# aelmiger/LINE-MOD-Pipeline

Hardware: AMD Instinct MI355X
Metric: detections/sec (higher is better)
Workload: dtype u8

## Files before the change

### line-mod-pipeline_amd/csrc/lm_common.h

```cpp
#pragma once
#include <stdint.h>

typedef uint8_t u8;
typedef uint16_t u16;
typedef uint32_t u32;
typedef uint64_t u64;

#define LM_SCAN_CHUNK 1008
#define LM_SCAN4_CHUNK 1016
#define LM_SCAN_FPAD 8
#define LM_SCANL_LDS_BYTES 163840
#define LM_SCANL_IMAGE_MAX 153600
#define LM_SCANL_TABLE_BYTES 2048
#define LM_SCANL_POS_BITS 15
#define LM_SORT_CAP 4096
#define LM_SORT_CHUNK 1024
#define LM_INLINE_MATCHES 2048
#define LM_DROPPED 0xFFFFFFFFu

#define PD_STRIP 16
#define CB_ROWS 2
#define CBS_STRIP 16
#define MX_WAVE_BYTES 128
#define CVT_ROWS 4
#define CG_STRIP 16
#define CT_W 32
#define CT_H 8
#define DT_W 64
#define DT_H 8
#define DM_ROWS 4
#ifndef DM_ROWS_BATCH
#define DM_ROWS_BATCH 16
#endif
#define LMK_MAX_LOADS 8

struct LmPhaseGrid { u32 nb[4]; int g[4]; };

struct LmLevelGeom {
    int w, h;
    int T;
    int W, H;
    int spread_only;
    int nibble;
    u32 wh;
    u32 ori_stride;
    u32 plane_ori;
    u32 mod_stride;
    u32 zero_off;
    u32 arena_bytes;
};

struct LmCand {
    u32 ti;
    int x, y;
    float sim;
};

struct LmRefFeat {
    u32 off;
    int16_t x, y;
};

struct LmRefMeta {
    int width, height;
    int nfeat_total;
// ... 55 lines not shown
```

### line-mod-pipeline_amd/csrc/lm_dev_depth.h

```cpp
#pragma once
#include "lm_dev.h"
#include "lm_median25.h"
#include "lm_median_counts.h"

namespace {

#define N_W (DT_W + 4)
#define N_H (DT_H + 4)
#define D_W (DT_W + 14)
#define D_H (DT_H + 14)
#define D_PITCH 80
#define D_LOADS ((D_H * D_W + 255) / 256)

typedef unsigned short us2 __attribute__((ext_vector_type(2)));
#define LM_CE(a, b) { us2 t_ = __builtin_elementwise_min(a, b); b = __builtin_elementwise_max(a, b); a = t_; }

__global__ __launch_bounds__(256) void k_depth_quantize(const u16* __restrict__ depth0, int w, int h, int dist_thr,
                                                         int diff_thr, const u8* __restrict__ lut,
                                                         u8* __restrict__ quant0, size_t slot_stride) {
    __shared__ u16 dt[D_H][D_PITCH];
    __shared__ u8 nt[N_H][N_W + 4];
    const u16* depth = slot_ptr(depth0, slot_stride);
    u8* quant = slot_ptr(quant0, slot_stride);
    const int tid = threadIdx.x;
// ... 197 lines not shown
    nx = nx * inv; ny = ny * inv; nz = nz * inv;
    const f32x2 t1 = nx * 10.f + 10.f, t2 = ny * 10.f + 10.f, t3 = nz * 20.f + 20.f;
    const u32 flat0 = (u32)mad_i24((int)t3[0], 400, mad_i24((int)t2[0], 20, (int)t1[0]));
    const u32 flat1 = (u32)mad_i24((int)t3[1], 400, mad_i24((int)t2[1], 20, (int)t1[1]));
    const u32 c0 = (u32)__builtin_amdgcn_raw_buffer_load_b8(lut_rsrc, (int)(LMK_NORMAL_CODE_OFFSET + min(flat0, 8000u)), 0, 0);
    const u32 c1 = (u32)__builtin_amdgcn_raw_buffer_load_b8(lut_rsrc, (int)(LMK_NORMAL_CODE_OFFSET + min(flat1, 8000u)), 0, 0);
    e0 = ok0 ? c0 : 0u; e1 = ok1 ? c1 : 0u;
}

__global__ __launch_bounds__(256) void k_selftest_float_tail(unsigned long long* __restrict__ out) {
    const u32 lo = 0x3F800000u, hi_rcp = (127u + 42u) << 23, hi_sqrt = (127u + 84u) << 23;
    unsigned long long bad_rcp = 0, bad_sqrt = 0, bad_bare = 0, c_rcp7 = 0, c_sqrt9 = 0, c_sqrt4 = 0, c_inv = 0;
    for (u32 b = lo + blockIdx.x * 256u + threadIdx.x; b <= hi_sqrt; b += gridDim.x * 256u) {
        const float x = __builtin_bit_cast(float, b);
        if (b <= hi_rcp) bad_rcp += __builtin_bit_cast(u32, dn_rcp(x)) != __builtin_bit_cast(u32, __fdiv_rn(1.0f, x));
        const u32 want = __builtin_bit_cast(u32, __builtin_sqrtf(x));
        bad_sqrt += __builtin_bit_cast(u32, dn_sqrt(x)) != want;
        bad_bare += __builtin_bit_cast(u32, dn_sqrt_bare(x)) != want;
        if (b <= hi_rcp) c_rcp7 += __builtin_bit_cast(u32, dn_rcp7(x)) != __builtin_bit_cast(u32, __fdiv_rn(1.0f, x));
        c_sqrt9 += __builtin_bit_cast(u32, dn_sqrt9(x)) != want;
        c_sqrt4 += __builtin_bit_cast(u32, dn_sqrt4(x)) != want;
        c_inv += __builtin_bit_cast(u32, dn_inv_from_rsq(x, dn_sqrt(x))) != __builtin_bit_cast(u32, __fdiv_rn(1.0f, __builtin_sqrtf(x)));
    }
    if (blockIdx.x == 0 && threadIdx.x == 0) bad_sqrt += dn_sqrt(0.0f) > 0.0f ? 1u : 0u;
    if (bad_rcp) atomicAdd(&out[0], bad_rcp);
    if (bad_sqrt) atomicAdd(&out[1], bad_sqrt);
    if (bad_bare) atomicAdd(&out[2], bad_bare);
    if (c_rcp7) atomicAdd(&out[3], c_rcp7);
    if (c_sqrt9) atomicAdd(&out[4], c_sqrt9);
    if (c_sqrt4) atomicAdd(&out[5], c_sqrt4);
    if (c_inv) atomicAdd(&out[6], c_inv);
}

template <bool SMALL>
__device__ __forceinline__ void d_dnormal_t(const u32 vblock, const u16* __restrict__ depth0, int w, int h, int dist_thr, int diff_thr,
                                                  const u8* __restrict__ lut, u8* __restrict__ code0, size_t in_stride,
                                                  size_t tmp_stride, int gblocks, int nslots) {
    u32 slot, tile;
    xcd_slot_tile_b(vblock, (u32)gblocks, (u32)nslots, slot, tile);
    const u16* depth = slot_ptr_s(depth0, in_stride, slot);
    u8* code = slot_ptr_s(code0, tmp_stride, slot);
    const int ng = w >> 3;
    const int gid = (int)(tile * 256u) + (int)threadIdx.x;
    const int y = gid / ng, g = gid - y * ng;
    if (y >= h) return;
    u32 out[2] = {0, 0};
    if (y >= 5 && y < h - 6) {
        u32x4 R[3][3];
#pragma unroll
        for (int j = 0; j < 3; ++j) {
            const u8* row = reinterpret_cast<const u8*>(depth + (size_t)(y + 5 * (j - 1)) * w) + 16 * g - 16;
#pragma unroll
            for (int k = 0; k < 3; ++k) {
                const bool ok = !(k == 0 && g == 0) && !(k == 2 && g == ng - 1);
                R[j][k] = ok ? ld16(row + 16 * k) : u32x4{0, 0, 0, 0};
            }
        }
        if (diff_thr >= 0 && diff_thr <= 5461) {
            const __amdgpu_buffer_rsrc_t lut_rsrc = __builtin_amdgcn_make_buffer_rsrc(const_cast<u8*>(lut), 0, 2 * 8000 + 16, 0x00020000);
            u32 D[3][12];
#pragma unroll
            for (int j = 0; j < 3; ++j)
#pragma unroll
                for (int k = 0; k < 12; ++k) D[j][k] = R[j][k >> 2][k & 3];
            const u32 THR = (u32)diff_thr * 0x00010001u;
#pragma unroll
            for (int k = 0; k < 4; ++k) {
                const u32 C = D[1][4 + k];
                u32 F[3][3], G[3][3];
#pragma unroll
                for (int jj = -1; jj <= 1; ++jj)
#pragma unroll
                    for (int ii = -1; ii <= 1; ++ii) {
                        if (ii == 0 && jj == 0) continue;
                        const u32* Dr = D[jj + 1];
                        const u32 N = ii == 0 ? Dr[4 + k]
                                    : ii > 0 ? __builtin_amdgcn_alignbit(Dr[7 + k], Dr[6 + k], 16)
                                             : __builtin_amdgcn_alignbit(Dr[2 + k], Dr[1 + k], 16);
                        const u32 up = pk_sub_u16_sat(N, C), dn = pk_sub_u16_sat(C, N);
                        const u32 f = pk_min_u16(pk_sub_u16_sat(THR, up | dn), 0x00010001u);
                        F[jj + 1][ii + 1] = f;
                        G[jj + 1][ii + 1] = pk_mul_lo_u16(pk_sub_i16(up, dn), f);
                    }
                const u32 fdp = F[2][2] + F[0][0], fdm = F[2][0] + F[0][2];
                const u32 cd = fdp + fdm;
                const u32 cx = pk_sub_i16(fdp, fdm);
                const u32 ci = F[1][2] + F[1][0] + cd, cj = F[2][1] + F[0][1] + cd;
                const u32 ga = pk_sub_i16(G[2][2], G[0][0]), gb = pk_sub_i16(G[0][2], G[2][0]);
                const u32 sx = pk_add_i16(pk_add_i16(pk_sub_i16(G[1][2], G[1][0]), ga), gb);
                const u32 sy = pk_sub_i16(pk_add_i16(pk_sub_i16(G[2][1], G[0][1]), ga), gb);
                const u32 ncx = pk_sub_i16(0u, cx);
                const int d0 = (int)(C & 0xFFFFu), d1 = (int)(C >> 16);
                const int detq0 = mad_i16h<false>(ci, cj, mad_i16h<false>(ncx, cx, 0)), detq1 = mad_i16h<true>(ci, cj, mad_i16h<true>(ncx, cx, 0));
                const int ddxq0 = mad_i16h<false>(cj, sx, mad_i16h<false>(ncx, sy, 0)), ddxq1 = mad_i16h<true>(cj, sx, mad_i16h<true>(ncx, sy, 0));
                const int ddyq0 = mad_i16h<false>(ci, sy, mad_i16h<false>(ncx, sx, 0)), ddyq1 = mad_i16h<true>(ci, sy, mad_i16h<true>(ncx, sx, 0));
                u32 e0, e1;
                dn_label2<SMALL>(detq0, ddxq0, ddyq0, d0, d0 < dist_thr, detq1, ddxq1, ddyq1, d1, d1 < dist_thr, lut_rsrc, e0, e1);
                out[k >> 1] |= (e0 | (e1 << 8)) << (16 * (k & 1));
            }
        } else {
#pragma unroll
        for (int p = 0; p < 8; ++p) {
            const int d = (int)hw_u16(R[1], 8 + p);
            const bool valid = d < dist_thr;
            int ci = 0, cj = 0, cx = 0, sx = 0, sy = 0;
#pragma unroll
            for (int jj = -1; jj <= 1; ++jj)
#pragma unroll
                for (int ii = -1; ii <= 1; ++ii) {
                    if (ii == 0 && jj == 0) continue;
                    const int delta = (int)hw_u16(R[jj + 1], 8 + p + 5 * ii) - d;
                    const int ad = delta < 0 ? -delta : delta;
                    const int f = ad < diff_thr ? 1 : 0;
                    const int fd = ad < diff_thr ? delta : 0;
                    if (ii != 0) { ci += f; sx += ii * fd; }
                    if (jj != 0) { cj += f; sy += jj * fd; }
                    if (ii != 0 && jj != 0) cx += ii * jj * f;
                }
            const int A0 = 25 * ci, A3 = 25 * cj, A1 = 25 * cx, b0 = 5 * sx, b1 = 5 * sy;
            const int det = mul_i24(A0, A3) - mul_i24(A1, A1);
            const int ddx = mul_i24(A3, b0) - mul_i24(A1, b1);
            const int ddy = mul_i24(A0, b1) - mul_i24(A1, b0);
            const u32 e = dn_label<false>(det, ddx, ddy, d, valid, lut);
            out[p >> 2] |= e << (8 * (p & 3));
        }
        }
    }
    {
        const int xlo = 5 - 8 * g, xhi = (w - 6) - 8 * g;
        unsigned long long m = ~0ull;
        if (xlo > 0) m &= xlo >= 8 ? 0ull : (~0ull << (8 * xlo));
        if (xhi < 8) m &= xhi <= 0 ? 0ull : (~0ull >> (8 * (8 - xhi)));
        out[0] &= (u32)m; out[1] &= (u32)(m >> 32);
    }
    *reinterpret_cast<u32x2*>(code + (size_t)y * w + 8 * g) = u32x2{out[0], out[1]};
}
__device__ __forceinline__ void d_dnormal(const u32 vblock, const u16* __restrict__ depth0, int w, int h, int dist_thr, int diff_thr,
                                          const u8* __restrict__ lut, u8* __restrict__ code0, size_t in_stride,
                                          size_t tmp_stride, int gblocks, int nslots) {
    if (diff_thr >= 0 && diff_thr <= 249) d_dnormal_t<true>(vblock, depth0, w, h, dist_thr, diff_thr, lut, code0, in_stride, tmp_stride, gblocks, nslots);
    else d_dnormal_t<false>(vblock, depth0, w, h, dist_thr, diff_thr, lut, code0, in_stride, tmp_stride, gblocks, nslots);
}
__global__ __launch_bounds__(256) void k_dnormal(const u16* __restrict__ depth0, int w, int h, int dist_thr, int diff_thr,
                                                  const u8* __restrict__ lut, u8* __restrict__ code0, size_t in_stride,
                                                  size_t tmp_stride, int gblocks, int nslots) {
    d_dnormal(blockIdx.x, depth0, w, h, dist_thr, diff_thr, lut, code0, in_stride, tmp_stride, gblocks, nslots);
}

template <int ROWS>
__device__ __forceinline__ void d_dmedian(const u32 vblock, const u8* __restrict__ code0, int w, int h, u8* __restrict__ quant0,
                                                  size_t tmp_stride, size_t out_stride, int gblocks, int nslots) {
    u32 slot, tile;
    xcd_slot_tile_b(vblock, (u32)gblocks, (u32)nslots, slot, tile);
    const u8* code = slot_ptr_s(code0, tmp_stride, slot);
    u8* quant = slot_ptr_s(quant0, out_stride, slot);
    const int ng = w >> 3;
    const int gid = (int)(tile * 256u) + (int)threadIdx.x;
    const int band = gid / ng, g = gid - band * ng;
    const int y0 = band * ROWS;
    if (y0 >= h) return;
    u32 ring[5][8];
#pragma unroll
    for (int i = 0; i < ROWS + 4; ++i) {
        const int yy = clampi(y0 - 2 + i, 0, h - 1);
        const u32 ro = (u32)yy * (u32)w + 8u * (u32)g;
        const u8* row = code + ro;
        const u32x2 c = *reinterpret_cast<const u32x2*>(row);
        u32 e[12];
#pragma unroll
        for (int k = 0; k < 8; ++k) e[2 + k] = (c[k >> 2] >> (8 * (k & 3))) & 0xFFu;
        const u32 l = *reinterpret_cast<const u32*>(code + (g > 0 ? ro - 4u : ro)), r = *reinterpret_cast<const u32*>(code + (g + 1 < ng ? ro + 8u : ro + 4u));
        e[0] = g > 0 ? (l >> 16) & 0xFFu : e[2]; e[1] = g > 0 ? l >> 24 : e[2];
        e[10] = g + 1 < ng ? r & 0xFFu : e[9]; e[11] = g + 1 < ng ? (r >> 8) & 0xFFu : e[9];
        u32 cw[12];
#pragma unroll
        for (int k = 0; k < 12; ++k) cw[k] = lm_mc_word(e[k]);
        u32 t3[10];
#pragma unroll
        for (int k = 0; k < 10; ++k) t3[k] = cw[k] + cw[k + 1] + cw[k + 2];
// ... 26 lines not shown
```

### line-mod-pipeline_amd/csrc/lm_host.cpp

```cpp
#include "lm_host.h"
#if defined(__x86_64__)
#include <immintrin.h>
#endif

#include <algorithm>
#include <atomic>
#include <cassert>
#include <cmath>
#include <cstdio>
#include <cstdlib>
#include <cstring>

namespace lmh {

int Bank::find(const std::string& id) const {
    for (size_t i = 0; i < classes.size(); ++i)
        if (classes[i].id == id) return (int)i;
    return -1;
}

int Bank::add_pyramid(const std::string& id, TemplatePyramid&& tp) {
    int ci = find(id);
    if (ci < 0) { classes.push_back(ClassEntry{id, {}}); ci = (int)classes.size() - 1; }
    classes[ci].pyramids.push_back(std::move(tp));
// ... 952 lines not shown
    const bool dep = in.M == 2;
    const int g_blur0 = cblur_blocks(w, h), g_blur1 = cblur_blocks(w1, h1);
    const int g_ori0 = corient_blocks(w, h), g_ori1 = corient_blocks(w1, h1);
    const int g_vote0 = cvote_blocks(w, h), g_vote1 = cvote_blocks(w1, h1);
    const int g_pyr = pyrdown8_blocks(w, h), g_nrm = dnormal_blocks(w, h), g_med = dmedian_blocks(w, h, DM_ROWS);
    const int seg0 = T0 == 5 ? lm_fast_segs(w / 5, 128) : lm_spread2_blocks(w, h), seg1 = lm_fast_segs(w1 / 8, 40);
    const u32 b_lm0 = T0 == 5 ? (u32)(seg0 * (h / 5) * n) : (u32)(seg0 * n), b_lm1 = (u32)(seg1 * (h1 / 8) * n);
    add_fused(p, K::Phase1, {{(u32)(g_blur0 * n), dep ? (u32)(g_nrm * n) : 0u, (u32)(g_pyr * n), 0u}, {g_blur0, g_nrm, g_pyr, 0}});
    add_fused(p, K::Phase2, {{dep ? (u32)(g_med * n) : 0u, (u32)(g_blur1 * n), (u32)(g_ori0 * n), 0u}, {g_med, g_blur1, g_ori0, 0}});
    add_fused(p, K::Phase3, {{(u32)(g_vote0 * n), (u32)(g_ori1 * n), dep ? b_lm0 : 0u, dep ? b_lm1 : 0u}, {g_vote0, g_ori1, seg0, seg1}});
    add_fused(p, T0 == 5 ? K::Phase4_T5 : K::Phase4_T2, {{(u32)(g_vote1 * n), b_lm0, 0u, 0u}, {g_vote1, seg0, 0, 0}});
    plan_mode_lm_fast(p, K::LmFast8_40, 40, 1, 0, false, in);
}

bool batch_phases_shape(const PreInputs& in) {
    if (!phases_shape(in) || !batch(in)) return false;
    if (in.lv[0].T == 5) return (in.lv[0].w % 5) == 0 && spread5_shape(in, 0, 0) && (in.M < 2 || spread5_shape(in, 0, 1));
    return in.M < 2;
}
void plan_batch_phases(const PreInputs& in, PrePlan& p) {
    const PreLevel &v0 = in.lv[0], &v1 = in.lv[1];
    const int w = v0.w, h = v0.h, w1 = w / 2, h1 = h / 2, n = in.n, T0 = v0.T;
    const bool tall = h > 640;
    const int sb = cblur_sh_strip(h);
    const int sg = tall ? 32 : 16;
    const int g_nrm = dnormal_blocks(w, h), g_blur0 = cblur_sh_blocks(w, h, sb), g_pyr = pyrdown16_blocks(w, h);
    const int g_grad0 = cgrad_blocks(w, h, sg), g_med = dmedian_blocks(w, h, DM_ROWS_BATCH), g_blur1 = cblur_sh_blocks(w1, h1, 16);
    const int g_grad1 = cgrad_blocks(w1, h1, 16);
    const int g_sp = T0 == 5 ? lm_spread5_blocks(w, h) : lm_spread2_blocks(w, h);
    const int seg1 = lm_fast_segs(w1 / 8, 40);
    const u32 b_lm1 = (u32)(seg1 * (h1 / 8) * n);
    if (in.M == 2) {
        if (plan_blur_pyrdown(in, p)) {
            add_slots(p, K::Dnormal, 0, 1, g_nrm, in);
        } else {
            add_fused(p, K::Bsplit0, {{(u32)(g_nrm * n), (u32)(g_pyr * n), 0u, 0u}, {g_nrm, g_pyr, 0, 0}});
            add_slots(p, tall ? K::CblurSh32 : K::CblurSh16, 0, 0, g_blur0, in);
        }
        add_fused(p, tall ? K::Bsplit1_32 : K::Bsplit1_16, {{(u32)(g_grad0 * n), (u32)(g_blur1 * n), 0u, 0u}, {g_grad0, g_blur1, 0, 0}});
        add_slots(p, K::Dmedian16, 0, 1, g_med, in);
        const int s1 = cgrad_strip_upper(w1, h1, n);
        add_slots(p, cgrad_kernel(s1), 1, 0, cgrad_blocks(w1, h1, s1), in);
        add_fused(p, K::Bsplit2, {{(u32)(g_sp * n), (u32)(g_sp * n), b_lm1, 0u}, {g_sp, g_sp, seg1, 0}});
    } else {
        const bool bp = plan_blur_pyrdown(in, p);
        static const K table[2][2][3] = {{{K::Bphase1_T5_16, K::Bphase2_T5_16, K::Bphase3_T5_16}, {K::Bphase1_T5_32, K::Bphase2_T5_32, K::Bphase3_T5_32}},
                                         {{K::Bphase1_T2_16, K::Bphase2_T2_16, K::Bphase3_T2_16}, {K::Bphase1_T2_32, K::Bphase2_T2_32, K::Bphase3_T2_32}}};
        const auto kern = [&](int ph) { return table[T0 == 5 ? 0 : 1][tall ? 1 : 0][ph - 1]; };
        if (!bp) add_fused(p, kern(1), {{0u, (u32)(g_blur0 * n), (u32)(g_pyr * n), 0u}, {g_nrm, g_blur0, g_pyr, 0}});
        add_fused(p, kern(2), {{(u32)(g_grad0 * n), 0u, (u32)(g_blur1 * n), 0u}, {g_grad0, g_med, g_blur1, 0}});
        add_fused(p, kern(3), {{(u32)(g_grad1 * n), (u32)(g_sp * n), 0u, 0u}, {g_grad1, g_sp, g_sp, seg1}});
    }
    const bool wide = lm_fast8_wide(w1 / 8, h1, v1.mode, v1.a_lm[0], in.a_stride, in.ori_stride, in.planes);
    plan_mode_lm_fast(p, wide ? K::LmFast8_80 : K::LmFast8_40, wide ? 80 : 40, 1, 0, false, in);
}

}

void plan_pyrdown(const PreInputs& in, int l, PrePlan& p) {
    const int sw = in.lv[l - 1].w, sh = in.lv[l - 1].h, v = in.knobs.pyrdown_variant;
    if (v != 1 && (v == 2 || batch(in)) && pyrdown16_shape(in, l)) add_slots(p, K::Pyrdown16, l, 0, pyrdown16_blocks(sw, sh), in);
    else if (pyrdown_streams(in, l)) add_slots(p, K::Pyrdown8, l, 0, pyrdown8_blocks(sw, sh), in);
    else add_tiles(p, K::Pyrdown, l, 0, pre_ceil(sw / 2, 64), pre_ceil(sh / 2, 4), in);
}

void plan_nn_half(const PreInputs& in, int l, PrePlan& p) { add_tiles(p, K::NnHalf, l, 1, pre_ceil(in.lv[l].w, 64), pre_ceil(in.lv[l].h, 4), in); }

void plan_color_quantize(const PreInputs& in, int l, bool blurred, PrePlan& p) {
    const int w = in.lv[l].w, h = in.lv[l].h, v = in.knobs.cgrad_variant;
    if (!color_streams(in, l)) { add_tiles(p, K::ColorQuantize, l, 0, pre_ceil(w, CT_W), pre_ceil(h, CT_H), in); return; }
    if (!blurred) add_blur(in, l, pick_blur(in, l), p);
    if (!in.want_mag && (v >= 2 || (v == 0 && batch(in)))) {
        const int strip = cgrad_strip(w, h, in.n, v == 3);
        add_slots(p, cgrad_kernel(strip), l, 0, cgrad_blocks(w, h, strip), in);
        return;
    }
    add_slots(p, K::Corient, l, 0, corient_blocks(w, h), in);
    add_slots(p, K::Cvote, l, 0, cvote_blocks(w, h), in);
}

void plan_depth_quantize(const PreInputs& in, PrePlan& p) {
    const int w = in.lv[0].w, h = in.lv[0].h, v = in.knobs.dmedian_variant;
    if (!depth_streams(in)) { add_tiles(p, K::DepthQuantize, 0, 1, pre_ceil(w, DT_W), pre_ceil(h, DT_H), in); return; }
    const bool dm_batch = v == 2 || (v == 0 && batch(in));
    add_slots(p, K::Dnormal, 0, 1, dnormal_blocks(w, h), in);
    add_slots(p, dm_batch ? K::Dmedian16 : K::Dmedian4, 0, 1, dmedian_blocks(w, h, dm_batch ? DM_ROWS_BATCH : DM_ROWS), in);
}

void plan_linear_memories(const PreInputs& in, int l, int m, u32 planes, PrePlan& p) {
    const PreLevel& v = in.lv[l];
    const bool sh = m != 0 && l != 0;
    const int w = v.w, h = v.h, T = v.T, W = w / T, mode = v.mode;
    const int qpitch = sh ? in.lv[l - 1].w : w;
    const u32 a_q = sh ? in.lv[l - 1].a_quant[1] : v.a_quant[m], a_lm = v.a_lm[m];
    if ((w % 4) == 0 && (W % 4) == 0 && (qpitch % 4) == 0 && (a_q & 3) == 0 && (in.a_stride & 3) == 0) {
        switch (T) {
            case 2:
                if (mode == 1 && !sh && (w % 32) == 0 && (h % 2) == 0 && (qpitch % 16) == 0 && a_q == 0 && a_lm == 0 && in.a_stride == 0 && (((size_t)W * (h / 2)) % 16) == 0) {
                    add_slots(p, K::LmSpread2, l, m, lm_spread2_blocks(w, h), in);
                    return;
                }
                plan_mode_lm_fast(p, K::LmFast2_128, 128, l, m, sh, in); return;
            case 4: plan_mode_lm_fast(p, K::LmFast4_64, 64, l, m, sh, in); return;
            case 5:
                if (mode == 1 && !sh && batch(in) && spread5_shape(in, l, m)) { add_slots(p, K::LmSpread5, l, m, lm_spread5_blocks(w, h), in); return; }
                plan_mode_lm_fast(p, K::LmFast5_128, 128, l, m, sh, in); return;
            case 8: {
                const bool wide = lm_fast8_wide(W, h, mode, a_lm, in.a_stride, in.ori_stride, planes);
                plan_mode_lm_fast(p, wide ? K::LmFast8_80 : K::LmFast8_40, wide ? 80 : 40, l, m, sh, in); return;
            }
            default: break;
        }
    }
    int seg = (1024 / (T * T)) & ~3;
    if (seg < 4) seg = 4;
    while (seg > 4 && (2 * T - 1) * (seg * T + T - 1) > LMK_MAX_LOADS * 256) seg -= 4;
    if (seg > W) seg = (W + 3) & ~3;
    const int pitch = (seg * T + T + 3) & ~3;
// ... 76 lines not shown
```

### line-mod-pipeline_amd/csrc/lm_k_preprocess.hip

```cpp
#include "lm_dev_color.h"
#include "lm_dev_depth.h"
#include "lm_dev_memories.h"
#include "lm_host.h"

namespace {

template <int PH, int T0>
__global__ __launch_bounds__(256) void k_phase(LmPhaseArgs a, LmPhaseGrid pg) {
    const u32 b = blockIdx.x, e0 = pg.nb[0], e1 = e0 + pg.nb[1], e2 = e1 + pg.nb[2];
    const size_t fs = a.slot_stride;
    const int w1 = a.w >> 1, h1 = a.h >> 1;
    const size_t a3_0 = ((size_t)a.w * a.h * 3 + 255) / 256 * 256, a3_1 = ((size_t)w1 * h1 * 3 + 255) / 256 * 256;
    const float thr2 = a.weak_threshold * a.weak_threshold;
    if (PH == 1) {
        if (b < e0) d_cblur(b, a.bgr0, a.w, a.h, a.cs0, fs, fs, pg.g[0], a.nslots);
        else if (b < e1) d_dnormal(b - e0, a.depth, a.w, a.h, a.dist_thr, a.diff_thr, a.normal_lut, a.ds, fs, fs, pg.g[1], a.nslots);
        else d_pyrdown8(b - e1, a.bgr0, a.w, a.h, a.bgr1, w1, h1, fs, pg.g[2], a.nslots);
    } else if (PH == 2) {
        if (b < e0) d_dmedian<DM_ROWS>(b, a.ds, a.w, a.h, a.qd0, fs, fs, pg.g[0], a.nslots);
        else if (b < e1) d_cblur(b - e0, a.bgr1, w1, h1, a.cs1, fs, fs, pg.g[1], a.nslots);
        else d_corient(b - e1, a.cs0, a.w, a.h, thr2, a.cs0 + a3_0, nullptr, fs, fs, pg.g[2], a.nslots);
    } else if (PH == 3) {
        if (b < e0) d_cvote(b, a.cs0 + a3_0, a.w, a.h, a.qc0, fs, fs, pg.g[0], a.nslots);
        else if (b < e1) d_corient(b - e0, a.cs1, w1, h1, thr2, a.cs1 + a3_1, nullptr, fs, fs, pg.g[1], a.nslots);
        else if (b < e2) d_lm_fast<5, 128, 0, 1>(b - e1, a.qd0, a.w, a.w, a.h, a.resp_tab, a.lm_d0, 0u, fs, fs, pg.g[2], a.nslots);
        else d_lm_fast<8, 40, 1, 2>(b - e2, a.qd0, a.w, w1, h1, a.resp_tab, a.lm_d1, a.ori_stride1, fs, fs, pg.g[3], a.nslots, a.plane_ori1);
    } else {
        if (b < e0) d_cvote(b, a.cs1 + a3_1, w1, h1, a.qc1, fs, fs, pg.g[0], a.nslots);
        else if (T0 == 5) d_lm_fast<5, 128, 0, 1>(b - e0, a.qc0, a.w, a.w, a.h, a.resp_tab, a.lm_c0, 0u, fs, fs, pg.g[1], a.nslots);
        else d_lm_spread2(b - e0, a.qc0, a.w, a.w, a.h, a.lm_c0, fs, fs, pg.g[1], a.nslots);
    }
}

template <int PH, int T0, int SB, int SG>
__global__ __launch_bounds__(256, 2) void k_bphase(LmPhaseArgs a, LmPhaseGrid pg) {
    const u32 b = blockIdx.x, e0 = pg.nb[0], e1 = e0 + pg.nb[1], e2 = e1 + pg.nb[2];
    const size_t fs = a.slot_stride;
    const int w1 = a.w >> 1, h1 = a.h >> 1, n = a.nslots;
    const float thr2 = a.weak_threshold * a.weak_threshold;
    const int ithr = thr2 >= 2147483648.f ? INT_MAX : (int)floorf(thr2);
    if (PH == 1) {
        if (b < e0) d_dnormal(b, a.depth, a.w, a.h, a.dist_thr, a.diff_thr, a.normal_lut, a.ds, fs, fs, pg.g[0], n);
        else if (b < e1) d_cblur_sh<SB>(b - e0, a.bgr0, a.w, a.h, a.cs0, fs, fs, pg.g[1], n);
        else d_pyrdown16<PD_STRIP>(b - e1, a.bgr0, a.w, a.h, a.bgr1, w1, h1, fs, pg.g[2], n);
    } else if (PH == 2) {
        if (b < e0) d_cgrad<SG>(b, a.cs0, a.w, a.h, ithr, a.qc0, fs, fs, pg.g[0], n);
        else if (b < e1) d_dmedian<DM_ROWS_BATCH>(b - e0, a.ds, a.w, a.h, a.qd0, fs, fs, pg.g[1], n);
        else d_cblur_sh<16>(b - e1, a.bgr1, w1, h1, a.cs1, fs, fs, pg.g[2], n);
    } else {
        if (b < e0) d_cgrad<16>(b, a.cs1, w1, h1, ithr, a.qc1, fs, fs, pg.g[0], n);
        else if (b < e1) {
            if (T0 == 5) d_lm_spread5(b - e0, a.qc0, a.w, a.w, a.h, a.lm_c0, fs, fs, pg.g[1], n);
            else d_lm_spread2(b - e0, a.qc0, a.w, a.w, a.h, a.lm_c0, fs, fs, pg.g[1], n);
        }
        else if (b < e2) d_lm_spread5(b - e1, a.qd0, a.w, a.w, a.h, a.lm_d0, fs, fs, pg.g[2], n);
        else d_lm_fast<8, 40, 1, 2>(b - e2, a.qd0, a.w, w1, h1, a.resp_tab, a.lm_d1, a.ori_stride1, fs, fs, pg.g[3], n, a.plane_ori1);
    }
}

template <int PART, int SG>
__global__ __launch_bounds__(256, PART == 1 ? 2 : 1) void k_bsplit(LmPhaseArgs a, LmPhaseGrid pg) {
    const u32 b = blockIdx.x, e0 = pg.nb[0], e1 = e0 + pg.nb[1];
    const size_t fs = a.slot_stride;
    const int w1 = a.w >> 1, h1 = a.h >> 1, n = a.nslots;
    if (PART == 0) {
        if (b < e0) d_dnormal(b, a.depth, a.w, a.h, a.dist_thr, a.diff_thr, a.normal_lut, a.ds, fs, fs, pg.g[0], n);
        else d_pyrdown16<PD_STRIP>(b - e0, a.bgr0, a.w, a.h, a.bgr1, w1, h1, fs, pg.g[1], n);
    } else if (PART == 1) {
        const float thr2 = a.weak_threshold * a.weak_threshold;
        const int ithr = thr2 >= 2147483648.f ? INT_MAX : (int)floorf(thr2);
        if (b < e0) d_cgrad<SG>(b, a.cs0, a.w, a.h, ithr, a.qc0, fs, fs, pg.g[0], n);
        else d_cblur_sh<16>(b - e0, a.bgr1, w1, h1, a.cs1, fs, fs, pg.g[1], n);
    } else {
        if (b < e0) d_lm_spread5(b, a.qc0, a.w, a.w, a.h, a.lm_c0, fs, fs, pg.g[0], n);
        else if (b < e1) d_lm_spread5(b - e0, a.qd0, a.w, a.w, a.h, a.lm_d0, fs, fs, pg.g[1], n);
        else d_lm_fast<8, 40, 1, 2>(b - e1, a.qd0, a.w, w1, h1, a.resp_tab, a.lm_d1, a.ori_stride1, fs, fs, pg.g[2], n, a.plane_ori1);
    }
}

__global__ void k_nn_half(const u8* __restrict__ src0, int sp, u8* __restrict__ dst0, int dw, int dh,
                          size_t slot_stride) {
    const u8* src = slot_ptr(src0, slot_stride);
    u8* dst = slot_ptr(dst0, slot_stride);
    int x = blockIdx.x * 64 + (threadIdx.x & 63), y = blockIdx.y * 4 + (threadIdx.x >> 6);
    if (x < dw && y < dh) dst[(size_t)y * dw + x] = src[(size_t)(2 * y) * sp + 2 * x];
}

}

size_t lmk_color_scratch_bytes(int w, int h) {
    size_t px = (size_t)w * h;
    return (px * 3 + 255) / 256 * 256 + (px + 255) / 256 * 256;
}

void lmk_preprocess_run(hipStream_t s, const lmh::PrePlan& p, int from, int to, const LmPreArgs& a) {
    typedef lmh::PreKernel K;
    const size_t fs = a.slot_stride;
    const int n = a.nslots;
    const float thr2 = a.weak_threshold * a.weak_threshold;
// ... 21 lines not shown
#define LM_FAST(T, SEG)                                                                                                              \
        do {                                                                                                                        \
            const int md = a.mode[l];                                                                                               \
            if (st.src_shift) { if (md == 1) LM_FAST_(T, SEG, 1, 1); else if (md == 2) LM_FAST_(T, SEG, 1, 2); else LM_FAST_(T, SEG, 1, 0); }   \
            else              { if (md == 1) LM_FAST_(T, SEG, 0, 1); else if (md == 2) LM_FAST_(T, SEG, 0, 2); else LM_FAST_(T, SEG, 0, 0); }   \
        } while (0)
#define LM_FAST_(T, SEG, SH, MD) LM_RUN((k_lm_fast<T, SEG, SH, MD>), q, qpitch, w, h, a.resp_tab, a.lm[l][m], a.ori_stride[l], fs, fs, g[0], n, planes)
#define LM_CGL(A, B) LM_RUN((k_cgrad_levels<A, B>), a.cs[0], a.w[0], a.h[0], a.quant[0][0], g[0], a.cs[1], a.w[1], a.h[1], a.quant[1][0], g[1], ithr, fs, n)
#define LM_FUSED(...) LM_RUN((__VA_ARGS__), pa, st.pg)
        switch (st.k) {
            case K::Pyrdown: LM_RUN(k_pyrdown, a.bgr[l - 1], a.w[l - 1], a.h[l - 1], a.bgr[l], a.w[l - 1] / 2, a.h[l - 1] / 2, fs); break;
            case K::Pyrdown8: LM_RUN(k_pyrdown8, a.bgr[l - 1], a.w[l - 1], a.h[l - 1], a.bgr[l], a.w[l - 1] / 2, a.h[l - 1] / 2, fs, g[0], n); break;
            case K::Pyrdown16: LM_RUN(k_pyrdown16<PD_STRIP>, a.bgr[l - 1], a.w[l - 1], a.h[l - 1], a.bgr[l], a.w[l - 1] / 2, a.h[l - 1] / 2, fs, g[0], n); break;
            case K::NnHalf: LM_RUN(k_nn_half, a.quant[l - 1][1], a.w[l - 1], a.quant[l][1], w, h, fs); break;
            case K::BlurPyr16: LM_RUN(k_blur_pyr<CBS_STRIP>, a.bgr[0], w, h, S, a.bgr[1], fs, g[0], g[1], n, st.param); break;
            case K::BlurPyr32: LM_RUN(k_blur_pyr<32>, a.bgr[0], w, h, S, a.bgr[1], fs, g[0], g[1], n, st.param); break;
            case K::BlurPyr64: LM_RUN(k_blur_pyr<64>, a.bgr[0], w, h, S, a.bgr[1], fs, g[0], g[1], n, st.param); break;
            case K::BlurMxPyr: LM_RUN(k_blur_mx_pyr, a.bgr[0], w, h, S, a.bgr[1], fs, g[0], g[1], st.param, g[2], n); break;
            case K::Cblur: LM_RUN(k_cblur, a.bgr[l], w, h, S, fs, fs, g[0], n); break;
            case K::CblurSh16: LM_RUN(k_cblur_sh<CBS_STRIP>, a.bgr[l], w, h, S, fs, fs, g[0], n); break;
            case K::CblurSh32: LM_RUN(k_cblur_sh<32>, a.bgr[l], w, h, S, fs, fs, g[0], n); break;
            case K::CblurMx: LM_RUN(k_cblur_mx, a.bgr[l], w, h, S, fs, fs, g[0], g[1], st.param, n); break;
            case K::Corient: LM_RUN(k_corient, S, w, h, thr2, S + qn_off, a.mag[l], fs, fs, g[0], n); break;
            case K::Cvote: LM_RUN(k_cvote, S + qn_off, w, h, a.quant[l][0], fs, fs, g[0], n); break;
            case K::Cgrad8: LM_RUN(k_cgrad<8>, S, w, h, ithr, a.quant[l][0], fs, fs, g[0], n); break;
            case K::Cgrad16: LM_RUN(k_cgrad<CG_STRIP>, S, w, h, ithr, a.quant[l][0], fs, fs, g[0], n); break;
            case K::Cgrad32: LM_RUN(k_cgrad<32>, S, w, h, ithr, a.quant[l][0], fs, fs, g[0], n); break;
            case K::ColorQuantize: LM_RUN(k_color_quantize, a.bgr[l], w, h, thr2, a.quant[l][0], a.mag[l], fs); break;
            case K::CgradLevels32_16: LM_CGL(32, 16); break;
            case K::CgradLevels32_8: LM_CGL(32, 8); break;
            case K::CgradLevels16_16: LM_CGL(CG_STRIP, 16); break;
            case K::CgradLevels16_8: LM_CGL(CG_STRIP, 8); break;
            case K::CgradLevels8_8: LM_CGL(8, 8); break;
            case K::Dnormal: LM_RUN(k_dnormal, a.depth, w, h, a.dist_thr, a.diff_thr, a.normal_lut, a.ds, fs, fs, g[0], n); break;
            case K::Dmedian4: LM_RUN(k_dmedian<DM_ROWS>, a.ds, w, h, a.quant[0][1], fs, fs, g[0], n); break;
            case K::Dmedian16: LM_RUN(k_dmedian<DM_ROWS_BATCH>, a.ds, w, h, a.quant[0][1], fs, fs, g[0], n); break;
            case K::DepthQuantize: LM_RUN(k_depth_quantize, a.depth, w, h, a.dist_thr, a.diff_thr, a.normal_lut, a.quant[0][1], fs); break;
            case K::MaskRules: case K::MatchMasks: break;
            case K::LmSpread2: LM_RUN(k_lm_spread2, q, qpitch, w, h, a.lm[l][m], fs, fs, g[0], n); break;
            case K::LmSpread5: LM_RUN(k_lm_spread5, q, qpitch, w, h, a.lm[l][m], fs, fs, g[0], n); break;
            case K::LmFast2_128: LM_FAST(2, 128); break;
            case K::LmFast4_64: LM_FAST(4, 64); break;
            case K::LmFast5_128: LM_FAST(5, 128); break;
            case K::LmFast8_40: LM_FAST(8, 40); break;
            case K::LmFast8_80: LM_FAST(8, 80); break;
            case K::LinearMemories:
                if (st.src_shift) { if (a.mode[l] == 1) LM_RUN((k_linear_memories<1, true>), q, qpitch, w, h, a.T[l], st.param, a.resp_tab, a.lm[l][m], a.ori_stride[l], fs, fs);
                                    else LM_RUN((k_linear_memories<1, false>), q, qpitch, w, h, a.T[l], st.param, a.resp_tab, a.lm[l][m], a.ori_stride[l], fs, fs); }
                else              { if (a.mode[l] == 1) LM_RUN((k_linear_memories<0, true>), q, qpitch, w, h, a.T[l], st.param, a.resp_tab, a.lm[l][m], a.ori_stride[l], fs, fs);
                                    else LM_RUN((k_linear_memories<0, false>), q, qpitch, w, h, a.T[l], st.param, a.resp_tab, a.lm[l][m], a.ori_stride[l], fs, fs); }
                break;
            case K::Phase1: LM_FUSED(k_phase<1, 5>); break;
            case K::Phase2: LM_FUSED(k_phase<2, 5>); break;
            case K::Phase3: LM_FUSED(k_phase<3, 5>); break;
            case K::Phase4_T5: LM_FUSED(k_phase<4, 5>); break;
            case K::Phase4_T2: LM_FUSED(k_phase<4, 2>); break;
            case K::Bsplit0: LM_FUSED(k_bsplit<0, 16>); break;
            case K::Bsplit1_16: LM_FUSED(k_bsplit<1, 16>); break;
            case K::Bsplit1_32: LM_FUSED(k_bsplit<1, 32>); break;
            case K::Bsplit2: LM_FUSED(k_bsplit<2, 16>); break;
            case K::Bphase1_T5_16: LM_FUSED(k_bphase<1, 5, 16, 16>); break;
            case K::Bphase2_T5_16: LM_FUSED(k_bphase<2, 5, 16, 16>); break;
            case K::Bphase3_T5_16: LM_FUSED(k_bphase<3, 5, 16, 16>); break;
            case K::Bphase1_T5_32: LM_FUSED(k_bphase<1, 5, 32, 32>); break;
            case K::Bphase2_T5_32: LM_FUSED(k_bphase<2, 5, 32, 32>); break;
            case K::Bphase3_T5_32: LM_FUSED(k_bphase<3, 5, 32, 32>); break;
            case K::Bphase1_T2_16: LM_FUSED(k_bphase<1, 2, 16, 16>); break;
// ... 19 lines not shown
```

Measured before the change: 201,900.

## Walk depth-normal rows in strips, reusing loaded neighbor rows and gates

The depth normal kernel changes from one output row per thread to a walk down a strip of rows spaced five apart. The loaded neighbor rows rotate through a three-row register ring, and the vertical gate values are carried forward. This cuts redundant global loads and gate computation. The cost is fewer active threads per launch, more serial work per thread and higher register pressure, with the strip length chosen per path (8 in batch mode, 1 otherwise).

Measured after the change: 205,300 (median of 6 runs). 1.02x the previous value.

```diff
diff --git a/line-mod-pipeline_amd/csrc/lm_common.h b/line-mod-pipeline_amd/csrc/lm_common.h
--- a/line-mod-pipeline_amd/csrc/lm_common.h
+++ b/line-mod-pipeline_amd/csrc/lm_common.h
@@ -31,6 +31,10 @@
 #define DM_ROWS 4
 #ifndef DM_ROWS_BATCH
 #define DM_ROWS_BATCH 16
+#endif
+#define DN_STRIP_FEW 1
+#ifndef DN_STRIP
+#define DN_STRIP 8
 #endif
 #define LMK_MAX_LOADS 8
 
diff --git a/line-mod-pipeline_amd/csrc/lm_dev_depth.h b/line-mod-pipeline_amd/csrc/lm_dev_depth.h
--- a/line-mod-pipeline_amd/csrc/lm_dev_depth.h
+++ b/line-mod-pipeline_amd/csrc/lm_dev_depth.h
@@ -253,119 +253,172 @@
     if (c_inv) atomicAdd(&out[6], c_inv);
 }
 
+__device__ __forceinline__ void dn_row_pixels(const u16* __restrict__ depth, int w, int g, int ng, int y, int dist_thr, int diff_thr,
+                                              const u8* __restrict__ lut, u32 (&out)[2]) {
+    u32x4 R[3][3];
+#pragma unroll
+    for (int j = 0; j < 3; ++j) {
+        const u8* row = reinterpret_cast<const u8*>(depth + (size_t)(y + 5 * (j - 1)) * w) + 16 * g - 16;
+#pragma unroll
+        for (int k = 0; k < 3; ++k) {
+            const bool ok = !(k == 0 && g == 0) && !(k == 2 && g == ng - 1);
+            R[j][k] = ok ? ld16(row + 16 * k) : u32x4{0, 0, 0, 0};
+        }
+    }
+#pragma unroll
+    for (int p = 0; p < 8; ++p) {
+        const int d = (int)hw_u16(R[1], 8 + p);
+        const bool valid = d < dist_thr;
+        int ci = 0, cj = 0, cx = 0, sx = 0, sy = 0;
+#pragma unroll
+        for (int jj = -1; jj <= 1; ++jj)
+#pragma unroll
+            for (int ii = -1; ii <= 1; ++ii) {
+                if (ii == 0 && jj == 0) continue;
+                const int delta = (int)hw_u16(R[jj + 1], 8 + p + 5 * ii) - d;
+                const int ad = delta < 0 ? -delta : delta;
+                const int f = ad < diff_thr ? 1 : 0;
+                const int fd = ad < diff_thr ? delta : 0;
+                if (ii != 0) { ci += f; sx += ii * fd; }
+                if (jj != 0) { cj += f; sy += jj * fd; }
+                if (ii != 0 && jj != 0) cx += ii * jj * f;
+            }
+        const int A0 = 25 * ci, A3 = 25 * cj, A1 = 25 * cx, b0 = 5 * sx, b1 = 5 * sy;
+        const int det = mul_i24(A0, A3) - mul_i24(A1, A1);
+        const int ddx = mul_i24(A3, b0) - mul_i24(A1, b1);
+        const int ddy = mul_i24(A0, b1) - mul_i24(A1, b0);
+        const u32 e = dn_label<false>(det, ddx, ddy, d, valid, lut);
+        out[p >> 2] |= e << (8 * (p & 3));
+    }
+}
+
+struct DnRow { u32 L[4], C[4], R[4]; };
+struct DnRaw { u32 a1, a2, a3; u32x4 b; u32 c0, c1, c2; };
+__device__ __forceinline__ DnRaw dn_load_row(const u8* __restrict__ db, u32 ro, u32 off_l, u32 off_r) {
+    DnRaw r;
+    ld12a4(db + (u32)(ro + off_l), r.a1, r.a2, r.a3); r.b = ld16(db + ro); ld12a4(db + (u32)(ro + off_r), r.c0, r.c1, r.c2);
+    return r;
+}
+__device__ __forceinline__ void dn_unpack_row(const DnRaw& r, DnRow& o) {
+    const u32 D[10] = {r.a1, r.a2, r.a3, r.b[0], r.b[1], r.b[2], r.b[3], r.c0, r.c1, r.c2};
+#pragma unroll
+    for (int k = 0; k < 4; ++k) {
+        o.C[k] = D[3 + k];
+        o.L[k] = __builtin_amdgcn_alignbit(D[1 + k], D[k], 16);
+        o.R[k] = __builtin_amdgcn_alignbit(D[6 + k], D[5 + k], 16);
+    }
+}
+__device__ __forceinline__ void dn_gate(u32 N, u32 C, u32 THR, u32& f, u32& g) {
+    const u32 up = pk_sub_u16_sat(N, C), dn = pk_sub_u16_sat(C, N);
+    f = pk_min_u16(pk_sub_u16_sat(THR, up | dn), 0x00010001u);
+    g = pk_mul_lo_u16(pk_sub_i16(up, dn), f);
+}
+template <bool SMALL>
+__device__ __forceinline__ void dn_step(const DnRow& m, const DnRow& c, const DnRow& p, u32 (&fv)[4], u32 (&gv)[4], u32 THR, int dist_thr,
+                                        const __amdgpu_buffer_rsrc_t lut_rsrc, u32 (&out)[2]) {
+#pragma unroll
+    for (int k = 0; k < 4; ++k) {
+        const u32 C = c.C[k];
+        u32 F[3][3], G[3][3];
+        dn_gate(m.L[k], C, THR, F[0][0], G[0][0]); dn_gate(m.R[k], C, THR, F[0][2], G[0][2]);
+        dn_gate(c.L[k], C, THR, F[1][0], G[1][0]); dn_gate(c.R[k], C, THR, F[1][2], G[1][2]);
+        dn_gate(p.L[k], C, THR, F[2][0], G[2][0]); dn_gate(p.C[k], C, THR, F[2][1], G[2][1]); dn_gate(p.R[k], C, THR, F[2][2], G[2][2]);
+        F[0][1] = fv[k];
+        const u32 fdp = F[2][2] + F[0][0], fdm = F[2][0] + F[0][2];
+        const u32 cd = fdp + fdm;
+        const u32 cx = pk_sub_i16(fdp, fdm);
+        const u32 ci = F[1][2] + F[1][0] + cd, cj = F[2][1] + F[0][1] + cd;
+        const u32 ga = pk_sub_i16(G[2][2], G[0][0]), gb = pk_sub_i16(G[0][2], G[2][0]);
+        const u32 sx = pk_add_i16(pk_add_i16(pk_sub_i16(G[1][2], G[1][0]), ga), gb);
+        const u32 sy = pk_sub_i16(pk_add_i16(pk_add_i16(G[2][1], gv[k]), ga), gb);
+        fv[k] = F[2][1]; gv[k] = G[2][1];
+        const u32 ncx = pk_sub_i16(0u, cx);
+        const int d0 = (int)(C & 0xFFFFu), d1 = (int)(C >> 16);
+        const int detq0 = mad_i16h<false>(ci, cj, mad_i16h<false>(ncx, cx, 0)), detq1 = mad_i16h<true>(ci, cj, mad_i16h<true>(ncx, cx, 0));
+        const int ddxq0 = mad_i16h<false>(cj, sx, mad_i16h<false>(ncx, sy, 0)), ddxq1 = mad_i16h<true>(cj, sx, mad_i16h<true>(ncx, sy, 0));
+        const int ddyq0 = mad_i16h<false>(ci, sy, mad_i16h<false>(ncx, sx, 0)), ddyq1 = mad_i16h<true>(ci, sy, mad_i16h<true>(ncx, sx, 0));
+        u32 e0, e1;
+        dn_label2<SMALL>(detq0, ddxq0, ddyq0, d0, d0 < dist_thr, detq1, ddxq1, ddyq1, d1, d1 < dist_thr, lut_rsrc, e0, e1);
+        out[k >> 1] |= (e0 | (e1 << 8)) << (16 * (k & 1));
+    }
+}
+
 template <bool SMALL>
 __device__ __forceinline__ void d_dnormal_t(const u32 vblock, const u16* __restrict__ depth0, int w, int h, int dist_thr, int diff_thr,
                                                   const u8* __restrict__ lut, u8* __restrict__ code0, size_t in_stride,
-                                                  size_t tmp_stride, int gblocks, int nslots) {
+                                                  size_t tmp_stride, int gblocks, int nslots, const int steps) {
     u32 slot, tile;
     xcd_slot_tile_b(vblock, (u32)gblocks, (u32)nslots, slot, tile);
     const u16* depth = slot_ptr_s(depth0, in_stride, slot);
     u8* code = slot_ptr_s(code0, tmp_stride, slot);
     const int ng = w >> 3;
+    if (steps * ((int)(tile * 256u) - 5 * ng) >= h * ng) return;
     const int gid = (int)(tile * 256u) + (int)threadIdx.x;
-    const int y = gid / ng, g = gid - y * ng;
+    const int q = gid / ng, g = gid - q * ng;
+    const int strip = q / 5, r = q - strip * 5;
+    int y = strip * (5 * steps) + r;
     if (y >= h) return;
-    u32 out[2] = {0, 0};
-    if (y >= 5 && y < h - 6) {
-        u32x4 R[3][3];
-#pragma unroll
-        for (int j = 0; j < 3; ++j) {
-            const u8* row = reinterpret_cast<const u8*>(depth + (size_t)(y + 5 * (j - 1)) * w) + 16 * g - 16;
-#pragma unroll
-            for (int k = 0; k < 3; ++k) {
-                const bool ok = !(k == 0 && g == 0) && !(k == 2 && g == ng - 1);
-                R[j][k] = ok ? ld16(row + 16 * k) : u32x4{0, 0, 0, 0};
-            }
-        }
-        if (diff_thr >= 0 && diff_thr <= 5461) {
-            const __amdgpu_buffer_rsrc_t lut_rsrc = __builtin_amdgcn_make_buffer_rsrc(const_cast<u8*>(lut), 0, 2 * 8000 + 16, 0x00020000);
-            u32 D[3][12];
-#pragma unroll
-            for (int j = 0; j < 3; ++j)
-#pragma unroll
-                for (int k = 0; k < 12; ++k) D[j][k] = R[j][k >> 2][k & 3];
-            const u32 THR = (u32)diff_thr * 0x00010001u;
-#pragma unroll
-            for (int k = 0; k < 4; ++k) {
-                const u32 C = D[1][4 + k];
-                u32 F[3][3], G[3][3];
-#pragma unroll
-                for (int jj = -1; jj <= 1; ++jj)
-#pragma unroll
-                    for (int ii = -1; ii <= 1; ++ii) {
-                        if (ii == 0 && jj == 0) continue;
-                        const u32* Dr = D[jj + 1];
-                        const u32 N = ii == 0 ? Dr[4 + k]
-                                    : ii > 0 ? __builtin_amdgcn_alignbit(Dr[7 + k], Dr[6 + k], 16)
-                                             : __builtin_amdgcn_alignbit(Dr[2 + k], Dr[1 + k], 16);
-                        const u32 up = pk_sub_u16_sat(N, C), dn = pk_sub_u16_sat(C, N);
-                        const u32 f = pk_min_u16(pk_sub_u16_sat(THR, up | dn), 0x00010001u);
-                        F[jj + 1][ii + 1] = f;
-                        G[jj + 1][ii + 1] = pk_mul_lo_u16(pk_sub_i16(up, dn), f);
-                    }
-                const u32 fdp = F[2][2] + F[0][0], fdm = F[2][0] + F[0][2];
-                const u32 cd = fdp + fdm;
-                const u32 cx = pk_sub_i16(fdp, fdm);
-                const u32 ci = F[1][2] + F[1][0] + cd, cj = F[2][1] + F[0][1] + cd;
-                const u32 ga = pk_sub_i16(G[2][2], G[0][0]), gb = pk_sub_i16(G[0][2], G[2][0]);
-                const u32 sx = pk_add_i16(pk_add_i16(pk_sub_i16(G[1][2], G[1][0]), ga), gb);
-                const u32 sy = pk_sub_i16(pk_add_i16(pk_sub_i16(G[2][1], G[0][1]), ga), gb);
-                const u32 ncx = pk_sub_i16(0u, cx);
-                const int d0 = (int)(C & 0xFFFFu), d1 = (int)(C >> 16);
-                const int detq0 = mad_i16h<false>(ci, cj, mad_i16h<false>(ncx, cx, 0)), detq1 = mad_i16h<true>(ci, cj, mad_i16h<true>(ncx, cx, 0));
-                const int ddxq0 = mad_i16h<false>(cj, sx, mad_i16h<false>(ncx, sy, 0)), ddxq1 = mad_i16h<true>(cj, sx, mad_i16h<true>(ncx, sy, 0));
-                const int ddyq0 = mad_i16h<false>(ci, sy, mad_i16h<false>(ncx, sx, 0)), ddyq1 = mad_i16h<true>(ci, sy, mad_i16h<true>(ncx, sx, 0));
-                u32 e0, e1;
-                dn_label2<SMALL>(detq0, ddxq0, ddyq0, d0, d0 < dist_thr, detq1, ddxq1, ddyq1, d1, d1 < dist_thr, lut_rsrc, e0, e1);
-                out[k >> 1] |= (e0 | (e1 << 8)) << (16 * (k & 1));
-            }
-        } else {
-#pragma unroll
-        for (int p = 0; p < 8; ++p) {
-            const int d = (int)hw_u16(R[1], 8 + p);
-            const bool valid = d < dist_thr;
-            int ci = 0, cj = 0, cx = 0, sx = 0, sy = 0;
-#pragma unroll
-            for (int jj = -1; jj <= 1; ++jj)
-#pragma unroll
-                for (int ii = -1; ii <= 1; ++ii) {
-                    if (ii == 0 && jj == 0) continue;
-                    const int delta = (int)hw_u16(R[jj + 1], 8 + p + 5 * ii) - d;
-                    const int ad = delta < 0 ? -delta : delta;
-                    const int f = ad < diff_thr ? 1 : 0;
-                    const int fd = ad < diff_thr ? delta : 0;
-                    if (ii != 0) { ci += f; sx += ii * fd; }
-                    if (jj != 0) { cj += f; sy += jj * fd; }
-                    if (ii != 0 && jj != 0) cx += ii * jj * f;
-                }
-            const int A0 = 25 * ci, A3 = 25 * cj, A1 = 25 * cx, b0 = 5 * sx, b1 = 5 * sy;
-            const int det = mul_i24(A0, A3) - mul_i24(A1, A1);
-            const int ddx = mul_i24(A3, b0) - mul_i24(A1, b1);
-            const int ddy = mul_i24(A0, b1) - mul_i24(A1, b0);
-            const u32 e = dn_label<false>(det, ddx, ddy, d, valid, lut);
-            out[p >> 2] |= e << (8 * (p & 3));
-        }
-        }
-    }
+    const int yend = min(h, (strip + 1) * (5 * steps));
+    const int ylast = min(yend, h - 6);
+    unsigned long long xm = ~0ull;
     {
         const int xlo = 5 - 8 * g, xhi = (w - 6) - 8 * g;
-        unsigned long long m = ~0ull;
-        if (xlo > 0) m &= xlo >= 8 ? 0ull : (~0ull << (8 * xlo));
-        if (xhi < 8) m &= xhi <= 0 ? 0ull : (~0ull >> (8 * (8 - xhi)));
-        out[0] &= (u32)m; out[1] &= (u32)(m >> 32);
-    }
-    *reinterpret_cast<u32x2*>(code + (size_t)y * w + 8 * g) = u32x2{out[0], out[1]};
+        if (xlo > 0) xm &= xlo >= 8 ? 0ull : (~0ull << (8 * xlo));
+        if (xhi < 8) xm &= xhi <= 0 ? 0ull : (~0ull >> (8 * (8 - xhi)));
+    }
+    const u32 xm0 = (u32)xm, xm1 = (u32)(xm >> 32);
+    const u32 co = 8u * (u32)g;
+    for (int yy = y; yy < yend; yy += 5)
+        if (yy < 5 || yy >= ylast) *reinterpret_cast<u32x2*>(code + ((u32)yy * (u32)w + co)) = u32x2{0, 0};
+    if (y < 5) y += 5;
+    if (y >= ylast) return;
+    u32 cofs = (u32)y * (u32)w + co;
+    const u32 clast = (u32)ylast * (u32)w;
+    if (diff_thr >= 0 && diff_thr <= 5461) {
+        const __amdgpu_buffer_rsrc_t lut_rsrc = __builtin_amdgcn_make_buffer_rsrc(const_cast<u8*>(lut), 0, 2 * 8000 + 16, 0x00020000);
+        const u32 THR = (u32)diff_thr * 0x00010001u;
+        const u8* db = reinterpret_cast<const u8*>(depth);
+        const u32 rb5 = 10u * (u32)w;
+        const u32 off_l = g == 0 ? 4u : 0u - 12u, off_r = g == ng - 1 ? 0u : 16u;
+        DnRow A, B, P;
+        dn_unpack_row(dn_load_row(db, 2u * cofs - rb5, off_l, off_r), A);
+        dn_unpack_row(dn_load_row(db, 2u * cofs, off_l, off_r), B);
+        u32 fv[4], gv[4];
+#pragma unroll
+        for (int k = 0; k < 4; ++k) dn_gate(B.C[k], A.C[k], THR, fv[k], gv[k]);
+#define DN_WALK_STEP(M, C, N)                                                                                   \
+        {                                                                                                       \
+            dn_unpack_row(dn_load_row(db, 2u * cofs + rb5, off_l, off_r), N);              \
+            u32 out[2] = {0, 0};                                                                                \
+            dn_step<SMALL>(M, C, N, fv, gv, THR, dist_thr, lut_rsrc, out);                                      \
+            *reinterpret_cast<u32x2*>(code + cofs) = u32x2{out[0] & xm0, out[1] & xm1};                         \
+            cofs += 5u * (u32)w;                                                                                \
+            if (cofs >= clast) break;                                                                           \
+        }
+        for (;;) {
+            DN_WALK_STEP(A, B, P)
+            DN_WALK_STEP(B, P, A)
+            DN_WALK_STEP(P, A, B)
+        }
+#undef DN_WALK_STEP
+    } else {
+        for (; cofs < clast; cofs += 5u * (u32)w, y += 5) {
+            u32 out[2] = {0, 0};
+            dn_row_pixels(depth, w, g, ng, y, dist_thr, diff_thr, lut, out);
+            *reinterpret_cast<u32x2*>(code + cofs) = u32x2{out[0] & xm0, out[1] & xm1};
+        }
+    }
 }
 __device__ __forceinline__ void d_dnormal(const u32 vblock, const u16* __restrict__ depth0, int w, int h, int dist_thr, int diff_thr,
                                           const u8* __restrict__ lut, u8* __restrict__ code0, size_t in_stride,
-                                          size_t tmp_stride, int gblocks, int nslots) {
-    if (diff_thr >= 0 && diff_thr <= 249) d_dnormal_t<true>(vblock, depth0, w, h, dist_thr, diff_thr, lut, code0, in_stride, tmp_stride, gblocks, nslots);
-    else d_dnormal_t<false>(vblock, depth0, w, h, dist_thr, diff_thr, lut, code0, in_stride, tmp_stride, gblocks, nslots);
+                                          size_t tmp_stride, int gblocks, int nslots, int steps) {
+    if (diff_thr >= 0 && diff_thr <= 249) d_dnormal_t<true>(vblock, depth0, w, h, dist_thr, diff_thr, lut, code0, in_stride, tmp_stride, gblocks, nslots, steps);
+    else d_dnormal_t<false>(vblock, depth0, w, h, dist_thr, diff_thr, lut, code0, in_stride, tmp_stride, gblocks, nslots, steps);
 }
 __global__ __launch_bounds__(256) void k_dnormal(const u16* __restrict__ depth0, int w, int h, int dist_thr, int diff_thr,
                                                   const u8* __restrict__ lut, u8* __restrict__ code0, size_t in_stride,
-                                                  size_t tmp_stride, int gblocks, int nslots) {
-    d_dnormal(blockIdx.x, depth0, w, h, dist_thr, diff_thr, lut, code0, in_stride, tmp_stride, gblocks, nslots);
+                                                  size_t tmp_stride, int gblocks, int nslots, int steps) {
+    d_dnormal(blockIdx.x, depth0, w, h, dist_thr, diff_thr, lut, code0, in_stride, tmp_stride, gblocks, nslots, steps);
 }
 
 template <int ROWS>
diff --git a/line-mod-pipeline_amd/csrc/lm_host.cpp b/line-mod-pipeline_amd/csrc/lm_host.cpp
--- a/line-mod-pipeline_amd/csrc/lm_host.cpp
+++ b/line-mod-pipeline_amd/csrc/lm_host.cpp
@@ -1008,7 +1008,7 @@
     const u32 b_lm1 = (u32)(seg1 * (h1 / 8) * n);
     if (in.M == 2) {
         if (plan_blur_pyrdown(in, p)) {
-            add_slots(p, K::Dnormal, 0, 1, g_nrm, in);
+            add_slots(p, K::Dnormal, 0, 1, g_nrm, in).pg.g[1] = DN_STRIP;
         } else {
             add_fused(p, K::Bsplit0, {{(u32)(g_nrm * n), (u32)(g_pyr * n), 0u, 0u}, {g_nrm, g_pyr, 0, 0}});
             add_slots(p, tall ? K::CblurSh32 : K::CblurSh16, 0, 0, g_blur0, in);
@@ -1059,7 +1059,8 @@
     const int w = in.lv[0].w, h = in.lv[0].h, v = in.knobs.dmedian_variant;
     if (!depth_streams(in)) { add_tiles(p, K::DepthQuantize, 0, 1, pre_ceil(w, DT_W), pre_ceil(h, DT_H), in); return; }
     const bool dm_batch = v == 2 || (v == 0 && batch(in));
-    add_slots(p, K::Dnormal, 0, 1, dnormal_blocks(w, h), in);
+    const int dn_steps = dm_batch ? DN_STRIP : DN_STRIP_FEW;
+    add_slots(p, K::Dnormal, 0, 1, dnormal_blocks(w, h), in).pg.g[1] = dn_steps;
     add_slots(p, dm_batch ? K::Dmedian16 : K::Dmedian4, 0, 1, dmedian_blocks(w, h, dm_batch ? DM_ROWS_BATCH : DM_ROWS), in);
 }
 
diff --git a/line-mod-pipeline_amd/csrc/lm_k_preprocess.hip b/line-mod-pipeline_amd/csrc/lm_k_preprocess.hip
--- a/line-mod-pipeline_amd/csrc/lm_k_preprocess.hip
+++ b/line-mod-pipeline_amd/csrc/lm_k_preprocess.hip
@@ -14,7 +14,7 @@
     const float thr2 = a.weak_threshold * a.weak_threshold;
     if (PH == 1) {
         if (b < e0) d_cblur(b, a.bgr0, a.w, a.h, a.cs0, fs, fs, pg.g[0], a.nslots);
-        else if (b < e1) d_dnormal(b - e0, a.depth, a.w, a.h, a.dist_thr, a.diff_thr, a.normal_lut, a.ds, fs, fs, pg.g[1], a.nslots);
+        else if (b < e1) d_dnormal(b - e0, a.depth, a.w, a.h, a.dist_thr, a.diff_thr, a.normal_lut, a.ds, fs, fs, pg.g[1], a.nslots, DN_STRIP_FEW);
         else d_pyrdown8(b - e1, a.bgr0, a.w, a.h, a.bgr1, w1, h1, fs, pg.g[2], a.nslots);
     } else if (PH == 2) {
         if (b < e0) d_dmedian<DM_ROWS>(b, a.ds, a.w, a.h, a.qd0, fs, fs, pg.g[0], a.nslots);
@@ -40,7 +40,7 @@
     const float thr2 = a.weak_threshold * a.weak_threshold;
     const int ithr = thr2 >= 2147483648.f ? INT_MAX : (int)floorf(thr2);
     if (PH == 1) {
-        if (b < e0) d_dnormal(b, a.depth, a.w, a.h, a.dist_thr, a.diff_thr, a.normal_lut, a.ds, fs, fs, pg.g[0], n);
+        if (b < e0) d_dnormal(b, a.depth, a.w, a.h, a.dist_thr, a.diff_thr, a.normal_lut, a.ds, fs, fs, pg.g[0], n, DN_STRIP);
         else if (b < e1) d_cblur_sh<SB>(b - e0, a.bgr0, a.w, a.h, a.cs0, fs, fs, pg.g[1], n);
         else d_pyrdown16<PD_STRIP>(b - e1, a.bgr0, a.w, a.h, a.bgr1, w1, h1, fs, pg.g[2], n);
     } else if (PH == 2) {
@@ -64,7 +64,7 @@
     const size_t fs = a.slot_stride;
     const int w1 = a.w >> 1, h1 = a.h >> 1, n = a.nslots;
     if (PART == 0) {
-        if (b < e0) d_dnormal(b, a.depth, a.w, a.h, a.dist_thr, a.diff_thr, a.normal_lut, a.ds, fs, fs, pg.g[0], n);
+        if (b < e0) d_dnormal(b, a.depth, a.w, a.h, a.dist_thr, a.diff_thr, a.normal_lut, a.ds, fs, fs, pg.g[0], n, DN_STRIP);
         else d_pyrdown16<PD_STRIP>(b - e0, a.bgr0, a.w, a.h, a.bgr1, w1, h1, fs, pg.g[1], n);
     } else if (PART == 1) {
         const float thr2 = a.weak_threshold * a.weak_threshold;
@@ -152,7 +152,7 @@
             case K::CgradLevels16_16: LM_CGL(CG_STRIP, 16); break;
             case K::CgradLevels16_8: LM_CGL(CG_STRIP, 8); break;
             case K::CgradLevels8_8: LM_CGL(8, 8); break;
-            case K::Dnormal: LM_RUN(k_dnormal, a.depth, w, h, a.dist_thr, a.diff_thr, a.normal_lut, a.ds, fs, fs, g[0], n); break;
+            case K::Dnormal: LM_RUN(k_dnormal, a.depth, w, h, a.dist_thr, a.diff_thr, a.normal_lut, a.ds, fs, fs, g[0], n, g[1]); break;
             case K::Dmedian4: LM_RUN(k_dmedian<DM_ROWS>, a.ds, w, h, a.quant[0][1], fs, fs, g[0], n); break;
             case K::Dmedian16: LM_RUN(k_dmedian<DM_ROWS_BATCH>, a.ds, w, h, a.quant[0][1], fs, fs, g[0], n); break;
             case K::DepthQuantize: LM_RUN(k_depth_quantize, a.depth, w, h, a.dist_thr, a.diff_thr, a.normal_lut, a.quant[0][1], fs); break;
```
